# lbcb-sci/herro

Hardware: NVIDIA H100
Metric: corrected_bases_per_sec (higher is better)
Workload: dtype u8 pileup/consensus + f32 forward

## Files before the change

herro_b200/csrc/gemm_tc.cu:

```cuda
#include <cstdio>
#include <cuda.h>
#include <cuda_bf16.h>

#include "common.cuh"
#include "forward.h"

namespace hb {

namespace {

constexpr int BM = 128, BN = 128, BK = 64, STAGES = 3;
constexpr int STAGE_BYTES = (2 * BM + 2 * BN) * 128;
constexpr int C_THREADS = 256, G_THREADS = 288, G_PROD_WARP = 8;

__device__ __forceinline__ uint32_t smem_u32(const void* p) { return (uint32_t)__cvta_generic_to_shared(p); }

__device__ __forceinline__ void mbar_init(uint64_t* bar, uint32_t count) {
    asm volatile("mbarrier.init.shared::cta.b64 [%0], %1;" ::"r"(smem_u32(bar)), "r"(count));
}
__device__ __forceinline__ void mbar_arrive(uint64_t* bar) {
    asm volatile("{\n\t.reg .b64 st;\n\tmbarrier.arrive.shared::cta.b64 st, [%0];\n\t}" ::"r"(smem_u32(bar)) : "memory");
}
__device__ __forceinline__ void mbar_wait(uint64_t* bar, uint32_t parity) {
    asm volatile(
        "{\n\t"
        ".reg .pred p;\n\t"
        "WAIT_LOOP:\n\t"
        "mbarrier.try_wait.parity.shared::cta.b64 p, [%0], %1;\n\t"
        "@p bra WAIT_DONE;\n\t"
        "bra WAIT_LOOP;\n\t"
        "WAIT_DONE:\n\t"
        "}" ::"r"(smem_u32(bar)), "r"(parity)
        : "memory");
}
__device__ __forceinline__ void mbar_arrive_expect_tx(uint64_t* bar, uint32_t bytes) {
    asm volatile("mbarrier.arrive.expect_tx.shared::cta.b64 _, [%0], %1;" ::"r"(smem_u32(bar)), "r"(bytes) : "memory");
}
__device__ __forceinline__ void tma_load_2d(uint32_t dst, const CUtensorMap* tm, uint64_t* bar, int c_inner, int c_row) {
    asm volatile("cp.async.bulk.tensor.2d.shared::cluster.global.mbarrier::complete_tx::bytes [%0], [%1, {%3, %4}], [%2];" ::"r"(dst),
                 "l"((uint64_t)tm), "r"(smem_u32(bar)), "r"(c_inner), "r"(c_row)
                 : "memory");
}
__device__ __forceinline__ void bar_sync(int id, int n) { asm volatile("bar.sync %0, %1;" ::"r"(id), "r"(n) : "memory"); }
__device__ __forceinline__ void fence_async_smem() { asm volatile("fence.proxy.async.shared::cta;" ::: "memory"); }

__device__ __forceinline__ uint64_t make_desc(uint32_t saddr) {
    uint64_t d = 0;
    d |= (uint64_t)((saddr & 0x3ffffu) >> 4);
    d |= (uint64_t)1 << 16;
    d |= (uint64_t)(1024u >> 4) << 32;
    d |= (uint64_t)1 << 62;
    return d;
}

__device__ __forceinline__ void wg_fence() { asm volatile("wgmma.fence.sync.aligned;" ::: "memory"); }
__device__ __forceinline__ void wg_commit() { asm volatile("wgmma.commit_group.sync.aligned;" ::: "memory"); }
template <int N>
__device__ __forceinline__ void wg_wait() { asm volatile("wgmma.wait_group.sync.aligned %0;" ::"n"(N) : "memory"); }
template <int R>
__device__ __forceinline__ void acc_fence(float (&a)[R]) {
#pragma unroll
    for (int i = 0; i < R; i++) asm volatile("" : "+f"(a[i])::"memory");
}

__device__ __forceinline__ void wgmma_n128(float (&d)[64], uint64_t adesc, uint64_t bdesc, uint32_t accumulate) {
    asm volatile(
        "{\n\t.reg .pred p;\n\tsetp.ne.b32 p, %66, 0;\n\t"
        "wgmma.mma_async.sync.aligned.m64n128k16.f32.bf16.bf16 "
        "{%0, %1, %2, %3, %4, %5, %6, %7, %8, %9, %10, %11, %12, %13, %14, %15, %16, %17, %18, %19, %20, %21, %22, %23, %24, %25, %26, %27, %28, %29, %30, %31, %32, %33, %34, %35, %36, %37, %38, %39, %40, %41, %42, %43, %44, %45, %46, %47, %48, %49, %50, %51, %52, %53, %54, %55, %56, %57, %58, %59, %60, %61, %62, %63}, "
        "%64, %65, p, 1, 1, 0, 0;\n\t}"
        : "+f"(d[0]), "+f"(d[1]), "+f"(d[2]), "+f"(d[3]), "+f"(d[4]), "+f"(d[5]), "+f"(d[6]), "+f"(d[7]), "+f"(d[8]), "+f"(d[9]), "+f"(d[10]), "+f"(d[11]), "+f"(d[12]), "+f"(d[13]), "+f"(d[14]), "+f"(d[15]), "+f"(d[16]), "+f"(d[17]), "+f"(d[18]), "+f"(d[19]), "+f"(d[20]), "+f"(d[21]), "+f"(d[22]), "+f"(d[23]), "+f"(d[24]), "+f"(d[25]), "+f"(d[26]), "+f"(d[27]), "+f"(d[28]), "+f"(d[29]), "+f"(d[30]), "+f"(d[31]), "+f"(d[32]), "+f"(d[33]), "+f"(d[34]), "+f"(d[35]), "+f"(d[36]), "+f"(d[37]), "+f"(d[38]), "+f"(d[39]), "+f"(d[40]), "+f"(d[41]), "+f"(d[42]), "+f"(d[43]), "+f"(d[44]), "+f"(d[45]), "+f"(d[46]), "+f"(d[47]), "+f"(d[48]), "+f"(d[49]), "+f"(d[50]), "+f"(d[51]), "+f"(d[52]), "+f"(d[53]), "+f"(d[54]), "+f"(d[55]), "+f"(d[56]), "+f"(d[57]), "+f"(d[58]), "+f"(d[59]), "+f"(d[60]), "+f"(d[61]), "+f"(d[62]), "+f"(d[63])
        : "l"(adesc), "l"(bdesc), "r"(accumulate)
        : "memory");
}
__device__ __forceinline__ void wgmma_n96(float (&d)[48], uint64_t adesc, uint64_t bdesc, uint32_t accumulate) {
    asm volatile(
        "{\n\t.reg .pred p;\n\tsetp.ne.b32 p, %50, 0;\n\t"
        "wgmma.mma_async.sync.aligned.m64n96k16.f32.bf16.bf16 "
        "{%0, %1, %2, %3, %4, %5, %6, %7, %8, %9, %10, %11, %12, %13, %14, %15, %16, %17, %18, %19, %20, %21, %22, %23, %24, %25, %26, %27, %28, %29, %30, %31, %32, %33, %34, %35, %36, %37, %38, %39, %40, %41, %42, %43, %44, %45, %46, %47}, "
        "%48, %49, p, 1, 1, 0, 0;\n\t}"
        : "+f"(d[0]), "+f"(d[1]), "+f"(d[2]), "+f"(d[3]), "+f"(d[4]), "+f"(d[5]), "+f"(d[6]), "+f"(d[7]), "+f"(d[8]), "+f"(d[9]), "+f"(d[10]), "+f"(d[11]), "+f"(d[12]), "+f"(d[13]), "+f"(d[14]), "+f"(d[15]), "+f"(d[16]), "+f"(d[17]), "+f"(d[18]), "+f"(d[19]), "+f"(d[20]), "+f"(d[21]), "+f"(d[22]), "+f"(d[23]), "+f"(d[24]), "+f"(d[25]), "+f"(d[26]), "+f"(d[27]), "+f"(d[28]), "+f"(d[29]), "+f"(d[30]), "+f"(d[31]), "+f"(d[32]), "+f"(d[33]), "+f"(d[34]), "+f"(d[35]), "+f"(d[36]), "+f"(d[37]), "+f"(d[38]), "+f"(d[39]), "+f"(d[40]), "+f"(d[41]), "+f"(d[42]), "+f"(d[43]), "+f"(d[44]), "+f"(d[45]), "+f"(d[46]), "+f"(d[47])
        : "l"(adesc), "l"(bdesc), "r"(accumulate)
        : "memory");
}

__device__ __forceinline__ void mma_kblock(float (&acc)[64], uint32_t a_hi, uint32_t a_lo, uint32_t b_hi, uint32_t b_lo, bool zero) {
    const uint64_t dAh = make_desc(a_hi), dAl = make_desc(a_lo), dBh = make_desc(b_hi), dBl = make_desc(b_lo);
    wg_fence();
#pragma unroll
    for (int k = 0; k < BK / 16; k++) {
        const uint64_t adv = (uint64_t)(k * 2);
        wgmma_n128(acc, dAh + adv, dBh + adv, (zero && k == 0) ? 0u : 1u);
        wgmma_n128(acc, dAl + adv, dBh + adv, 1u);
        wgmma_n128(acc, dAh + adv, dBl + adv, 1u);
    }
    wg_commit();
}

__device__ __forceinline__ void split2(float a, float b, uint32_t& hi, uint32_t& lo) {
    const __nv_bfloat162 h = __floats2bfloat162_rn(a, b);
    hi = *reinterpret_cast<const uint32_t*>(&h);
    const float ah = __uint_as_float(hi << 16), bh = __uint_as_float(hi & 0xffff0000u);
    const __nv_bfloat162 l = __floats2bfloat162_rn(a - ah, b - bh);
    lo = *reinterpret_cast<const uint32_t*>(&l);
}

__device__ __forceinline__ void frag_ln_stats(const float (&a)[64], float& m0, float& r0, float& m1, float& r1) {
    float s0 = 0.f, s1 = 0.f;
#pragma unroll
    for (int j = 0; j < 16; j++) { s0 += a[4 * j] + a[4 * j + 1]; s1 += a[4 * j + 2] + a[4 * j + 3]; }
    s0 += __shfl_xor_sync(HB_FULL, s0, 1); s0 += __shfl_xor_sync(HB_FULL, s0, 2);
    s1 += __shfl_xor_sync(HB_FULL, s1, 1); s1 += __shfl_xor_sync(HB_FULL, s1, 2);
    m0 = s0 * (1.f / BN); m1 = s1 * (1.f / BN);
    float v0 = 0.f, v1 = 0.f;
#pragma unroll
    for (int j = 0; j < 16; j++) {
        float d = a[4 * j] - m0; v0 = fmaf(d, d, v0);
        d = a[4 * j + 1] - m0; v0 = fmaf(d, d, v0);
        d = a[4 * j + 2] - m1; v1 = fmaf(d, d, v1);
        d = a[4 * j + 3] - m1; v1 = fmaf(d, d, v1);
    }
    v0 += __shfl_xor_sync(HB_FULL, v0, 1); v0 += __shfl_xor_sync(HB_FULL, v0, 2);
    v1 += __shfl_xor_sync(HB_FULL, v1, 1); v1 += __shfl_xor_sync(HB_FULL, v1, 2);
    r0 = rsqrtf(v0 * (1.f / BN) + 1e-5f); r1 = rsqrtf(v1 * (1.f / BN) + 1e-5f);
}
__device__ __forceinline__ void frag_layernorm(float (&a)[64], const float* gam, const float* bet, int fc) {
    float m0, r0, m1, r1;
    frag_ln_stats(a, m0, r0, m1, r1);
#pragma unroll
    for (int j = 0; j < 16; j++) {
        const int c = 8 * j + fc;
        const float g0 = gam[c], g1 = gam[c + 1], b0 = bet[c], b1 = bet[c + 1];
        a[4 * j] = (a[4 * j] - m0) * r0 * g0 + b0;
        a[4 * j + 1] = (a[4 * j + 1] - m0) * r0 * g1 + b1;
        a[4 * j + 2] = (a[4 * j + 2] - m1) * r1 * g0 + b0;
        a[4 * j + 3] = (a[4 * j + 3] - m1) * r1 * g1 + b1;
    }
}
__device__ __forceinline__ void frag_store_f32(const float (&a)[64], float* base, size_t ld, size_t row0, int c0, int fc) {
#pragma unroll
    for (int j = 0; j < 16; j++) {
        *(float2*)(base + row0 * ld + c0 + 8 * j + fc) = make_float2(a[4 * j], a[4 * j + 1]);
        *(float2*)(base + (row0 + 8) * ld + c0 + 8 * j + fc) = make_float2(a[4 * j + 2], a[4 * j + 3]);
    }
}
__device__ __forceinline__ void frag_store_split(const float (&a)[64], __nv_bfloat16* hi, __nv_bfloat16* lo, size_t ld, size_t row0, int c0,
                                                 int fc) {
#pragma unroll
    for (int j = 0; j < 16; j++) {
        uint32_t h, l;
        const size_t o0 = row0 * ld + c0 + 8 * j + fc, o1 = (row0 + 8) * ld + c0 + 8 * j + fc;
        split2(a[4 * j], a[4 * j + 1], h, l);
        *(uint32_t*)(hi + o0) = h; *(uint32_t*)(lo + o0) = l;
        split2(a[4 * j + 2], a[4 * j + 3], h, l);
        *(uint32_t*)(hi + o1) = h; *(uint32_t*)(lo + o1) = l;
    }
}
__device__ __forceinline__ void frag_store_tile(const float (&a)[64], uint8_t* tile, int r, int fc, const float* gam = nullptr,
                                                const float* bet = nullptr, const float* ln = nullptr) {
#pragma unroll
    for (int j = 0; j < 16; j++)
#pragma unroll
        for (int hf = 0; hf < 2; hf++) {
            const int rr = r + 8 * hf, c = 8 * j + fc;
            float x = a[4 * j + 2 * hf], y = a[4 * j + 2 * hf + 1];
            if (gam) {
                x = (x - ln[2 * hf]) * ln[2 * hf + 1] * gam[c] + bet[c];
                y = (y - ln[2 * hf]) * ln[2 * hf + 1] * gam[c + 1] + bet[c + 1];
            }
            uint32_t h, l;
            split2(x, y, h, l);
            const uint32_t off = (uint32_t)(j >> 3) * (2 * BM * 128) + (uint32_t)rr * 128u + (uint32_t)((((j & 7) ^ (rr & 7)) << 4) + fc * 2);
            *(uint32_t*)(tile + off) = h;
            *(uint32_t*)(tile + off + BM * 128) = l;
        }
}

}

__global__ void __launch_bounds__(G_THREADS, 1) k_gemm_ws(GemmArgs g, const __grid_constant__ CUtensorMap tmAhi,
                                                         const __grid_constant__ CUtensorMap tmAlo, const __grid_constant__ CUtensorMap tmWhi,
                                                         const __grid_constant__ CUtensorMap tmWlo) {
    extern __shared__ uint8_t smem_dyn[];
    uint8_t* smem = smem_dyn + ((1024u - (smem_u32(smem_dyn) & 1023u)) & 1023u);
    __shared__ uint64_t full_bar[STAGES], empty_bar[STAGES];
    __shared__ __align__(16) float s_lng[BN], s_lnb[BN];

    const int tid = threadIdx.x, warp = tid >> 5, lane = tid & 31;
    if (tid == 0) {
        for (int s = 0; s < STAGES; s++) { mbar_init(&full_bar[s], 1); mbar_init(&empty_bar[s], C_THREADS); }
        asm volatile("fence.mbarrier_init.release.cluster;" ::: "memory");
    }
    if (g.mode == GEMM_OUT_F32_RES_LN && tid < BN) { s_lng[tid] = g.ln_g[tid]; s_lnb[tid] = g.ln_b[tid]; }
    __syncthreads();

    const uint32_t n_items = g.m_tiles * g.n_chunks;
    const uint32_t kbs = g.k_blocks;

    if (warp == G_PROD_WARP) {
        if (lane == 0) {
            uint32_t it_stage = 0;
            for (uint32_t item = blockIdx.x; item < n_items; item += gridDim.x) {
                const int m0 = (int)((item / g.n_chunks) * BM), n0 = (int)((item % g.n_chunks) * BN);
                for (uint32_t kb = 0; kb < kbs; kb++, it_stage++) {
                    const uint32_t s = it_stage % STAGES, ph = (it_stage / STAGES) & 1;
                    mbar_wait(&empty_bar[s], ph ^ 1);
                    const uint32_t sb = smem_u32(smem + (size_t)s * STAGE_BYTES);
                    const int k0 = (int)(kb * BK);
                    mbar_arrive_expect_tx(&full_bar[s], STAGE_BYTES);
                    tma_load_2d(sb, &tmAhi, &full_bar[s], k0, m0);
                    tma_load_2d(sb + BM * 128, &tmAlo, &full_bar[s], k0, m0);
                    tma_load_2d(sb + 2 * BM * 128, &tmWhi, &full_bar[s], k0, n0);
                    tma_load_2d(sb + 2 * BM * 128 + BN * 128, &tmWlo, &full_bar[s], k0, n0);
                }
            }
        }
        return;
    }
    const int wg = warp >> 2;
    const int fr = wg * 64 + (warp & 3) * 16 + (lane >> 2), fc = (lane & 3) * 2;
    uint32_t it_stage = 0;
    float acc[64];
    for (uint32_t item = blockIdx.x; item < n_items; item += gridDim.x) {
        const uint32_t m0 = (item / g.n_chunks) * BM, n0 = (item % g.n_chunks) * BN;
        uint32_t prev = 0;
        for (uint32_t kb = 0; kb < kbs; kb++, it_stage++) {
            const uint32_t s = it_stage % STAGES, ph = (it_stage / STAGES) & 1;
            mbar_wait(&full_bar[s], ph);
            const uint32_t sb = smem_u32(smem + (size_t)s * STAGE_BYTES);
            mma_kblock(acc, sb + wg * 64 * 128, sb + BM * 128 + wg * 64 * 128, sb + 2 * BM * 128, sb + 2 * BM * 128 + BN * 128, kb == 0);
            if (kb > 0) {
                wg_wait<1>();
                mbar_arrive(&empty_bar[prev]);
            }
            prev = s;
        }
        wg_wait<0>();
        acc_fence(acc);
        mbar_arrive(&empty_bar[prev]);
        const size_t row0 = (size_t)m0 + fr;
        if (g.mode == GEMM_OUT_F32_RES_LN) {
#pragma unroll
            for (int j = 0; j < 16; j++) {
                const int c = 8 * j + fc;
                const float2 bv = *(const float2*)(g.bias + c);
                const float2 x0 = *(const float2*)(g.res + row0 * g.ldc + c), x1 = *(const float2*)(g.res + (row0 + 8) * g.ldc + c);
                acc[4 * j] = acc[4 * j] + bv.x + x0.x; acc[4 * j + 1] = acc[4 * j + 1] + bv.y + x0.y;
                acc[4 * j + 2] = acc[4 * j + 2] + bv.x + x1.x; acc[4 * j + 3] = acc[4 * j + 3] + bv.y + x1.y;
            }
            frag_store_f32(acc, g.out, g.ldc, row0, 0, fc);
            frag_layernorm(acc, s_lng, s_lnb, fc);
            frag_store_split(acc, g.out_hi, g.out_lo, g.ldo, row0, 0, fc);
            continue;
        }
#pragma unroll
        for (int j = 0; j < 16; j++) {
            const int c = (int)n0 + 8 * j + fc;
            const float2 bv = *(const float2*)(g.bias + c);
            acc[4 * j] += bv.x; acc[4 * j + 1] += bv.y; acc[4 * j + 2] += bv.x; acc[4 * j + 3] += bv.y;
            if (g.mode == GEMM_OUT_F32_RES) {
                const float2 x0 = *(const float2*)(g.res + row0 * g.ldc + c), x1 = *(const float2*)(g.res + (row0 + 8) * g.ldc + c);
                acc[4 * j] += x0.x; acc[4 * j + 1] += x0.y; acc[4 * j + 2] += x1.x; acc[4 * j + 3] += x1.y;
            } else if (g.mode == GEMM_OUT_F32_RELU || g.mode == GEMM_OUT_SPLIT_RELU) {
#pragma unroll
                for (int e = 0; e < 4; e++) acc[4 * j + e] = fmaxf(acc[4 * j + e], 0.f);
            }
        }
        if (g.mode == GEMM_OUT_SPLIT_RELU) frag_store_split(acc, g.out_hi, g.out_lo, g.ldo, row0, (int)n0, fc);
        else frag_store_f32(acc, g.out, g.ldc, row0, (int)n0, fc);
    }
}

constexpr int FFN_RING_BYTES = 2 * BN * 128;
constexpr int FFN_A_BYTES = 2 * 2 * BM * 128;
constexpr int FFN_STAGES = 2;

template <bool FUSE_O>
__global__ void __launch_bounds__(G_THREADS, 1) k_ffn_ws(FfnArgs g, const __grid_constant__ CUtensorMap tmHhi,
                                                        const __grid_constant__ CUtensorMap tmHlo, const __grid_constant__ CUtensorMap tmW1hi,
                                                        const __grid_constant__ CUtensorMap tmW1lo, const __grid_constant__ CUtensorMap tmW2hi,
                                                        const __grid_constant__ CUtensorMap tmW2lo, const __grid_constant__ CUtensorMap tmWohi,
                                                        const __grid_constant__ CUtensorMap tmWolo) {
    extern __shared__ uint8_t smem_dyn[];
    uint8_t* smem = smem_dyn + ((1024u - (smem_u32(smem_dyn) & 1023u)) & 1023u);
    uint8_t* sA1 = smem;
    uint8_t* sA2 = sA1 + FFN_A_BYTES;
    uint8_t* ring = sA2 + FFN_A_BYTES;
    __shared__ uint64_t full_bar[FFN_STAGES], empty_bar[FFN_STAGES], a1_full, a1_empty;
    __shared__ __align__(16) float s_b1[512], s_b2[BN], s_lng[BN], s_lnb[BN], s_bo[BN], s_ln2g[BN], s_ln2b[BN];

    const int tid = threadIdx.x, warp = tid >> 5, lane = tid & 31;
    if (tid == 0) {
        for (int s = 0; s < FFN_STAGES; s++) { mbar_init(&full_bar[s], 1); mbar_init(&empty_bar[s], C_THREADS); }
        mbar_init(&a1_full, 1); mbar_init(&a1_empty, C_THREADS);
        asm volatile("fence.mbarrier_init.release.cluster;" ::: "memory");
    }
    for (int i = tid; i < 512; i += G_THREADS) s_b1[i] = g.b1[i];
    if (tid < BN) { s_b2[tid] = g.b2[tid]; s_lng[tid] = g.ln_g[tid]; s_lnb[tid] = g.ln_b[tid]; }
    if (FUSE_O && tid < BN) { s_bo[tid] = g.bo[tid]; s_ln2g[tid] = g.ln2_g[tid]; s_ln2b[tid] = g.ln2_b[tid]; }
    __syncthreads();

    if (warp == G_PROD_WARP) {
        if (lane == 0) {
            uint32_t it_stage = 0, n_done = 0;
            auto load_w = [&](const CUtensorMap* hi, const CUtensorMap* lo, int col, int row) {
                const uint32_t s = it_stage % FFN_STAGES, ph = (it_stage / FFN_STAGES) & 1;
                mbar_wait(&empty_bar[s], ph ^ 1);
                const uint32_t sb = smem_u32(ring + (size_t)s * FFN_RING_BYTES);
                mbar_arrive_expect_tx(&full_bar[s], FFN_RING_BYTES);
                tma_load_2d(sb, hi, &full_bar[s], col, row);
                tma_load_2d(sb + BN * 128, lo, &full_bar[s], col, row);
                it_stage++;
            };
            for (uint32_t tile = blockIdx.x; tile < g.m_tiles; tile += gridDim.x, n_done++) {
                mbar_wait(&a1_empty, (n_done & 1) ^ 1);
                mbar_arrive_expect_tx(&a1_full, FFN_A_BYTES);
                for (int kb = 0; kb < 2; kb++) {
                    tma_load_2d(smem_u32(sA1) + kb * (2 * BM * 128), &tmHhi, &a1_full, kb * BK, (int)(tile * BM));
                    tma_load_2d(smem_u32(sA1) + kb * (2 * BM * 128) + BM * 128, &tmHlo, &a1_full, kb * BK, (int)(tile * BM));
                }
                if (FUSE_O)
                    for (int kb = 0; kb < 2; kb++) load_w(&tmWohi, &tmWolo, kb * BK, 0);
                for (int c = 0; c < 4; c++) {
                    for (int kb = 0; kb < 2; kb++) load_w(&tmW1hi, &tmW1lo, kb * BK, c * 128);
                    for (int kb = 0; kb < 2; kb++) load_w(&tmW2hi, &tmW2lo, c * 128 + kb * BK, 0);
                }
            }
        }
        return;
    }
    const int wg = warp >> 2;
    const int fr = wg * 64 + (warp & 3) * 16 + (lane >> 2), fc = (lane & 3) * 2;
    const uint32_t a1b = smem_u32(sA1) + wg * 64 * 128, a2b = smem_u32(sA2) + wg * 64 * 128;
    uint32_t it_stage = 0, n_done = 0;
    float accO[64], accF[64];
    auto contract = [&](float (&acc)[64], uint32_t abase, bool zero) {
        for (int kb = 0; kb < 2; kb++, it_stage++) {
            const uint32_t s = it_stage % FFN_STAGES, ph = (it_stage / FFN_STAGES) & 1;
            mbar_wait(&full_bar[s], ph);
            const uint32_t sb = smem_u32(ring + (size_t)s * FFN_RING_BYTES);
            const uint32_t a = abase + kb * (2 * BM * 128);
            mma_kblock(acc, a, a + BM * 128, sb, sb + BN * 128, zero && kb == 0);
        }
        wg_wait<0>();
        acc_fence(acc);
        mbar_arrive(&empty_bar[(it_stage - 2) % FFN_STAGES]);
        mbar_arrive(&empty_bar[(it_stage - 1) % FFN_STAGES]);
    };
    for (uint32_t tile = blockIdx.x; tile < g.m_tiles; tile += gridDim.x, n_done++) {
        const size_t row0 = (size_t)tile * BM + fr;
        if (!FUSE_O) {
#pragma unroll
            for (int j = 0; j < 16; j++) {
                const int c = 8 * j + fc;
                const float2 x0 = *(const float2*)(g.X + row0 * BN + c), x1 = *(const float2*)(g.X + (row0 + 8) * BN + c);
                accO[4 * j] = x0.x + s_b2[c]; accO[4 * j + 1] = x0.y + s_b2[c + 1];
                accO[4 * j + 2] = x1.x + s_b2[c]; accO[4 * j + 3] = x1.y + s_b2[c + 1];
            }
        }
        mbar_wait(&a1_full, n_done & 1);
        if (FUSE_O) {
            contract(accO, a1b, true);
#pragma unroll
            for (int j = 0; j < 16; j++) {
                const int c = 8 * j + fc;
                const float2 x0 = *(const float2*)(g.X + row0 * BN + c), x1 = *(const float2*)(g.X + (row0 + 8) * BN + c);
                accO[4 * j] = accO[4 * j] + s_bo[c] + x0.x; accO[4 * j + 1] = accO[4 * j + 1] + s_bo[c + 1] + x0.y;
                accO[4 * j + 2] = accO[4 * j + 2] + s_bo[c] + x1.x; accO[4 * j + 3] = accO[4 * j + 3] + s_bo[c + 1] + x1.y;
            }
            float ln[4];
            frag_ln_stats(accO, ln[0], ln[1], ln[2], ln[3]);
            bar_sync(1 + wg, 128);
            frag_store_tile(accO, sA1, fr, fc, s_ln2g, s_ln2b, ln);
#pragma unroll
            for (int j = 0; j < 16; j++) {
                const int c = 8 * j + fc;
                accO[4 * j] += s_b2[c]; accO[4 * j + 1] += s_b2[c + 1]; accO[4 * j + 2] += s_b2[c]; accO[4 * j + 3] += s_b2[c + 1];
            }
            fence_async_smem();
            bar_sync(1 + wg, 128);
        }
        for (int c = 0; c < 4; c++) {
            contract(accF, a1b, true);
            if (c == 3) mbar_arrive(&a1_empty);
#pragma unroll
            for (int j = 0; j < 16; j++) {
                const float b0 = s_b1[c * 128 + 8 * j + fc], b1 = s_b1[c * 128 + 8 * j + fc + 1];
                accF[4 * j] = fmaxf(accF[4 * j] + b0, 0.f); accF[4 * j + 1] = fmaxf(accF[4 * j + 1] + b1, 0.f);
                accF[4 * j + 2] = fmaxf(accF[4 * j + 2] + b0, 0.f); accF[4 * j + 3] = fmaxf(accF[4 * j + 3] + b1, 0.f);
            }
            frag_store_tile(accF, sA2, fr, fc);
            fence_async_smem();
            bar_sync(1 + wg, 128);
            contract(accO, a2b, false);
            bar_sync(1 + wg, 128);
        }
        if (g.store_x) frag_store_f32(accO, g.X, BN, row0, 0, fc);
        frag_layernorm(accO, s_lng, s_lnb, fc);
        frag_store_split(accO, g.out_hi, g.out_lo, BN, row0, 0, fc);
    }
}

constexpr int QA_HROWS = 96;
constexpr int QA_RING_BYTES = 2 * QA_HROWS * 128;
constexpr int QA_STAGES = 3;
constexpr int QA_POS_BYTES = 6 * 2048;

__device__ __forceinline__ void ldsm_x4(uint32_t addr, uint32_t (&r)[4]) {
    asm volatile("ldmatrix.sync.aligned.m8n8.x4.shared.b16 {%0, %1, %2, %3}, [%4];" : "=r"(r[0]), "=r"(r[1]), "=r"(r[2]), "=r"(r[3]) : "r"(addr));
}
__device__ __forceinline__ void ldsm_x4_trans(uint32_t addr, uint32_t (&r)[4]) {
    asm volatile("ldmatrix.sync.aligned.m8n8.x4.trans.shared.b16 {%0, %1, %2, %3}, [%4];" : "=r"(r[0]), "=r"(r[1]), "=r"(r[2]), "=r"(r[3]) : "r"(addr));
}
__device__ __forceinline__ void mma16816(float (&c)[4], const uint32_t (&a)[4], uint32_t b0, uint32_t b1) {
    asm volatile("mma.sync.aligned.m16n8k16.row.col.f32.bf16.bf16.f32 {%0, %1, %2, %3}, {%4, %5, %6, %7}, {%8, %9}, {%0, %1, %2, %3};"
                 : "+f"(c[0]), "+f"(c[1]), "+f"(c[2]), "+f"(c[3])
                 : "r"(a[0]), "r"(a[1]), "r"(a[2]), "r"(a[3]), "r"(b0), "r"(b1));
}
__device__ __forceinline__ uint32_t qa_off(int row, int chunk) { return (uint32_t)(row * 64 + ((chunk ^ ((row >> 1) & 3)) << 4)); }

__global__ void __launch_bounds__(G_THREADS, 1) k_qkv_attn_ws(QkvAttnArgs g, const __grid_constant__ CUtensorMap tmHhi,
                                                             const __grid_constant__ CUtensorMap tmHlo, const __grid_constant__ CUtensorMap tmWhi,
                                                             const __grid_constant__ CUtensorMap tmWlo) {
    extern __shared__ uint8_t smem_dyn[];
    uint8_t* smem = smem_dyn + ((1024u - (smem_u32(smem_dyn) & 1023u)) & 1023u);
    uint8_t* sA = smem;
    uint8_t* ring = sA + FFN_A_BYTES;
    uint8_t* sP = ring + QA_STAGES * QA_RING_BYTES;
    __shared__ uint64_t full_bar[QA_STAGES], empty_bar[QA_STAGES], a_full, a_empty;
    __shared__ __align__(16) float s_bias[4 * QA_HROWS];

    const int tid = threadIdx.x, warp = tid >> 5, lane = tid & 31;
    if (tid == 0) {
        for (int s = 0; s < QA_STAGES; s++) { mbar_init(&full_bar[s], 1); mbar_init(&empty_bar[s], C_THREADS); }
        mbar_init(&a_full, 1); mbar_init(&a_empty, C_THREADS);
        asm volatile("fence.mbarrier_init.release.cluster;" ::: "memory");
    }
    for (int i = tid; i < 4 * QA_HROWS; i += G_THREADS) s_bias[i] = g.bias[i];
    __syncthreads();

    if (warp == G_PROD_WARP) {
        if (lane == 0) {
            uint32_t it_stage = 0, n_done = 0;
            for (uint32_t tile = blockIdx.x; tile < g.m_tiles; tile += gridDim.x, n_done++) {
                const int m0 = (int)(tile * BM);
                mbar_wait(&a_empty, (n_done & 1) ^ 1);
                mbar_arrive_expect_tx(&a_full, FFN_A_BYTES);
                for (int kb = 0; kb < 2; kb++) {
                    tma_load_2d(smem_u32(sA) + kb * (2 * BM * 128), &tmHhi, &a_full, kb * BK, m0);
                    tma_load_2d(smem_u32(sA) + kb * (2 * BM * 128) + BM * 128, &tmHlo, &a_full, kb * BK, m0);
                }
                for (int h = 0; h < 4; h++)
                    for (int kb = 0; kb < 2; kb++, it_stage++) {
                        const uint32_t s = it_stage % QA_STAGES, ph = (it_stage / QA_STAGES) & 1;
                        mbar_wait(&empty_bar[s], ph ^ 1);
                        const uint32_t sb = smem_u32(ring + (size_t)s * QA_RING_BYTES);
                        mbar_arrive_expect_tx(&full_bar[s], QA_RING_BYTES);
                        tma_load_2d(sb, &tmWhi, &full_bar[s], kb * BK, h * QA_HROWS);
                        tma_load_2d(sb + QA_HROWS * 128, &tmWlo, &full_bar[s], kb * BK, h * QA_HROWS);
                    }
            }
        }
        return;
    }
    const int wg = warp >> 2;
    const int pos = wg * 2 + ((warp & 3) >> 1);
    const int mt = warp & 1;
    const int gq = lane >> 2, tq = lane & 3;
    uint8_t* pb = sP + (size_t)pos * QA_POS_BYTES;
    uint8_t *aQh = pb, *aQl = pb + 2048, *aKh = pb + 4096, *aKl = pb + 6144, *aVh = pb + 8192, *aVl = pb + 10240;
    const uint32_t uQh = smem_u32(aQh), uQl = smem_u32(aQl), uKh = smem_u32(aKh), uKl = smem_u32(aKl), uVh = smem_u32(aVh),
                   uVl = smem_u32(aVl);
    const float scale_l2 = rsqrtf(32.f) * 1.4426950408889634f;
    const uint32_t ab = smem_u32(sA) + wg * 64 * 128;
    uint32_t it_stage = 0, n_done = 0;
    for (uint32_t tile = blockIdx.x; tile < g.m_tiles; tile += gridDim.x, n_done++) {
        mbar_wait(&a_full, n_done & 1);
        for (int h = 0; h < 4; h++) {
            float acc[48];
            for (int kb = 0; kb < 2; kb++, it_stage++) {
                const uint32_t s = it_stage % QA_STAGES, ph = (it_stage / QA_STAGES) & 1;
                mbar_wait(&full_bar[s], ph);
                const uint32_t sb = smem_u32(ring + (size_t)s * QA_RING_BYTES);
                const uint32_t a = ab + kb * (2 * BM * 128);
                const uint64_t dAh = make_desc(a), dAl = make_desc(a + BM * 128), dBh = make_desc(sb), dBl = make_desc(sb + QA_HROWS * 128);
                wg_fence();
#pragma unroll
                for (int k = 0; k < BK / 16; k++) {
                    const uint64_t adv = (uint64_t)(k * 2);
                    wgmma_n96(acc, dAh + adv, dBh + adv, (kb | k) ? 1u : 0u);
                    wgmma_n96(acc, dAl + adv, dBh + adv, 1u);
                    wgmma_n96(acc, dAh + adv, dBl + adv, 1u);
                }
                wg_commit();
            }
            wg_wait<0>();
            acc_fence(acc);
            mbar_arrive(&empty_bar[(it_stage - 2) % QA_STAGES]);
            mbar_arrive(&empty_bar[(it_stage - 1) % QA_STAGES]);
            if (h == 3) mbar_arrive(&a_empty);
            bar_sync(3 + pos, 64);
            const float* bb = s_bias + h * QA_HROWS;
#pragma unroll
            for (int j = 0; j < 12; j++) {
                const int c = 8 * j + 2 * tq;
                const float sc = j < 4 ? scale_l2 : 1.f;
                uint8_t* hi_arr = j < 4 ? aQh : (j < 8 ? aKh : aVh);
                const int cc = c & 31;
#pragma unroll
                for (int hf = 0; hf < 2; hf++) {
                    const int row = mt * 16 + hf * 8 + gq;
                    uint32_t hw, lw;
                    split2((acc[4 * j + 2 * hf] + bb[c]) * sc, (acc[4 * j + 2 * hf + 1] + bb[c + 1]) * sc, hw, lw);
                    const uint32_t off = qa_off(row, cc >> 3) + (cc & 7) * 2;
                    *(uint32_t*)(hi_arr + off) = hw;
                    *(uint32_t*)(hi_arr + 2048 + off) = lw;
                }
            }
            bar_sync(3 + pos, 64);
            float sacc[4][4];
#pragma unroll
            for (int nt = 0; nt < 4; nt++)
#pragma unroll
                for (int e = 0; e < 4; e++) sacc[nt][e] = 0.f;
            {
                uint32_t qh[2][4], ql[2][4];
#pragma unroll
                for (int ks = 0; ks < 2; ks++) {
                    const uint32_t off = qa_off(mt * 16 + (lane & 7) + ((lane >> 3) & 1) * 8, ks * 2 + (lane >> 4));
                    ldsm_x4(uQh + off, qh[ks]);
                    ldsm_x4(uQl + off, ql[ks]);
                }
#pragma unroll
                for (int ntp = 0; ntp < 2; ntp++)
#pragma unroll
                    for (int ks = 0; ks < 2; ks++) {
                        uint32_t kh[4], kl[4];
                        const uint32_t off = qa_off(ntp * 16 + (lane & 7) + (lane >> 4) * 8, ks * 2 + ((lane >> 3) & 1));
                        ldsm_x4(uKh + off, kh);
                        ldsm_x4(uKl + off, kl);
#pragma unroll
                        for (int j = 0; j < 2; j++) {
                            mma16816(sacc[ntp * 2 + j], qh[ks], kh[2 * j], kh[2 * j + 1]);
                            mma16816(sacc[ntp * 2 + j], ql[ks], kh[2 * j], kh[2 * j + 1]);
                            mma16816(sacc[ntp * 2 + j], qh[ks], kl[2 * j], kl[2 * j + 1]);
                        }
                    }
            }
            float inv[2];
// ... 164 lines not shown
    if (warp >= S_GATHER_WARP) {
        const int gt = tid - S_GATHER_WARP * 32;
        uint32_t n_done = 0;
        for (uint32_t item = blockIdx.x; item < n_items; item += gridDim.x, n_done++) {
            uint8_t* tb = tokbuf + (n_done & 1) * 4 * STEM_MAXK * 32;
            uint8_t* qb = qbuf + (n_done & 1) * 4 * STEM_MAXK * 32;
            uint32_t m_row = 0, m_L = 0, m_Lref = 0;
            uint64_t m_base = 0;
            if (lane < 4 && item * 4 + lane < g.npos) {
                const uint32_t w = b.fwd_win[g.n0 + item * 4 + lane];
                m_row = b.fwd_row[g.n0 + item * 4 + lane];
                m_L = b.w_L[w]; m_Lref = b.w_reflmax[w]; m_base = b.w_rowbase[w];
            }
            mbar_wait(&buf_empty[n_done & 1], ((n_done >> 1) & 1) ^ 1);
            for (int i0 = 0; i0 < 4 * K * 2; i0 += S_GATHER) {
                const int i = i0 + gt;
                const int ps = min(i / (K * 2), 3), rem = i % (K * 2), j = rem >> 1, half = rem & 1;
                const uint32_t r = __shfl_sync(HB_FULL, m_row, ps), L = __shfl_sync(HB_FULL, m_L, ps), Lref = __shfl_sync(HB_FULL, m_Lref, ps);
                const uint64_t rbase = __shfl_sync(HB_FULL, m_base, ps);
                uint4 tv = make_uint4(0xffffffffu, 0xffffffffu, 0xffffffffu, 0xffffffffu), qv = make_uint4(0, 0, 0, 0);
                const int64_t row = (int64_t)r + j - K / 2;
                if (row >= 0 && row < (int64_t)Lref) {
                    if (row < (int64_t)L) {
                        const uint64_t off = (rbase + row) * ROW_BYTES + half * 16;
                        tv = *(const uint4*)(b.mat_bases + off);
                        qv = *(const uint4*)(b.mat_quals + off);
                    } else {
                        tv = make_uint4(0x0b0b0b0bu, 0x0b0b0b0bu, 0x0b0b0b0bu, 0x0b0b0b0bu);
                        qv = make_uint4(0x7e7e7e7eu, 0x7e7e7e7eu, 0x7e7e7e7eu, 0x7e7e7e7eu);
                    }
                }
                if (i < 4 * K * 2) {
                    *(uint4*)(tb + (ps * STEM_MAXK + j) * 32 + half * 16) = tv;
                    *(uint4*)(qb + (ps * STEM_MAXK + j) * 32 + half * 16) = qv;
                }
            }
            mbar_arrive(&buf_full[n_done & 1]);
        }
        return;
    }
    const int wg = warp >> 2;
    const int fr = wg * 64 + (warp & 3) * 16 + (lane >> 2), fc = (lane & 3) * 2;
    const int rd0 = fr & 31, rd1 = (fr + 8) & 31;
    uint32_t it_stage = 0;
    float acc[64];
    for (uint32_t item = blockIdx.x; item < n_items; item += gridDim.x) {
        uint32_t prev = 0;
        for (uint32_t kb = 0; kb < kbs; kb++, it_stage++) {
            const uint32_t s = it_stage % STAGES, ph = (it_stage / STAGES) & 1;
            mbar_wait(&full_bar[s], ph);
            const uint32_t sb = smem_u32(smem + (size_t)s * STEM_STAGE_BYTES);
            const uint64_t dA = make_desc(sb + wg * 64 * 128), dBh = make_desc(sb + BM * 128), dBl = make_desc(sb + BM * 128 + BN * 128);
            wg_fence();
#pragma unroll
            for (int k = 0; k < BK / 16; k++) {
                const uint64_t adv = (uint64_t)(k * 2);
                wgmma_n128(acc, dA + adv, dBh + adv, (kb | (uint32_t)k) ? 1u : 0u);
                wgmma_n128(acc, dA + adv, dBl + adv, 1u);
            }
            wg_commit();
            if (kb > 0) {
                wg_wait<1>();
                mbar_arrive(&empty_bar[prev]);
            }
            prev = s;
        }
        wg_wait<0>();
        acc_fence(acc);
        mbar_arrive(&empty_bar[prev]);
        const size_t row0 = (size_t)item * BM + fr;
#pragma unroll
        for (int j = 0; j < 16; j++) {
            const int c = 8 * j + fc;
            const float* rp0 = s_rp + rd0 * STEM_RP_LD + c;
            const float* rp1 = s_rp + rd1 * STEM_RP_LD + c;
            acc[4 * j] = fmaxf(acc[4 * j] + s_bias[c], 0.f) + rp0[0];
            acc[4 * j + 1] = fmaxf(acc[4 * j + 1] + s_bias[c + 1], 0.f) + rp0[1];
            acc[4 * j + 2] = fmaxf(acc[4 * j + 2] + s_bias[c], 0.f) + rp1[0];
            acc[4 * j + 3] = fmaxf(acc[4 * j + 3] + s_bias[c + 1], 0.f) + rp1[1];
            if (rd0 >= R_COLS) { acc[4 * j] = 0.f; acc[4 * j + 1] = 0.f; }
            if (rd1 >= R_COLS) { acc[4 * j + 2] = 0.f; acc[4 * j + 3] = 0.f; }
        }
        frag_store_f32(acc, g.X, BN, row0, 0, fc);
        if (g.out_hi) {
            frag_layernorm(acc, s_lng, s_lnb, fc);
            frag_store_split(acc, g.out_hi, g.out_lo, BN, row0, 0, fc);
        }
    }
}

__global__ void k_split_bf16(const float* __restrict__ w, __nv_bfloat16* __restrict__ hi, __nv_bfloat16* __restrict__ lo, size_t n) {
    const size_t i = (size_t)blockIdx.x * blockDim.x + threadIdx.x;
    if (i < n) {
        const __nv_bfloat16 h = __float2bfloat16_rn(w[i]);
        hi[i] = h;
        lo[i] = __float2bfloat16_rn(w[i] - __bfloat162float(h));
    }
}

cudaError_t split_weights(const float* w, size_t n, void** hi, void** lo) {
    cudaError_t e = cudaMalloc(hi, n * 2);
    if (e != cudaSuccess) return e;
    e = cudaMalloc(lo, n * 2);
    if (e != cudaSuccess) return e;
    k_split_bf16<<<(unsigned)((n + 255) / 256), 256>>>(w, (__nv_bfloat16*)*hi, (__nv_bfloat16*)*lo, n);
    return cudaGetLastError();
}

typedef CUresult (*EncodeTiledFn)(CUtensorMap*, CUtensorMapDataType, cuuint32_t, void*, const cuuint64_t*, const cuuint64_t*,
                                  const cuuint32_t*, const cuuint32_t*, CUtensorMapInterleave, CUtensorMapSwizzle,
                                  CUtensorMapL2promotion, CUtensorMapFloatOOBfill);
static EncodeTiledFn encode_fn() {
    static EncodeTiledFn fn = nullptr;
    if (!fn) {
        void* p = nullptr;
        cudaDriverEntryPointQueryResult q;
        if (cudaGetDriverEntryPoint("cuTensorMapEncodeTiled", &p, cudaEnableDefault, &q) == cudaSuccess) fn = (EncodeTiledFn)p;
    }
    return fn;
}
static bool make_tmap(CUtensorMap* tm, const void* base, uint64_t rows, uint64_t cols, uint64_t ld, uint32_t box_rows = BM) {
    EncodeTiledFn fn = encode_fn();
    if (!fn) return false;
    const cuuint64_t gdim[2] = {cols, rows};
    const cuuint64_t gstr[1] = {ld * 2};
    const cuuint32_t box[2] = {BK, box_rows};
    const cuuint32_t estr[2] = {1, 1};
    return fn(tm, CU_TENSOR_MAP_DATA_TYPE_BFLOAT16, 2, const_cast<void*>(base), gdim, gstr, box, estr, CU_TENSOR_MAP_INTERLEAVE_NONE,
              CU_TENSOR_MAP_SWIZZLE_128B, CU_TENSOR_MAP_L2_PROMOTION_L2_128B, CU_TENSOR_MAP_FLOAT_OOB_FILL_NONE) == CUDA_SUCCESS;
}

cudaError_t gemm_tc(const GemmArgs& a, int num_sms, cudaStream_t st) {
    static bool configured = false;
    const size_t smem = (size_t)STAGES * STAGE_BYTES + 1024;
    if (!configured) {
        cudaError_t e = cudaFuncSetAttribute(k_gemm_ws, cudaFuncAttributeMaxDynamicSharedMemorySize, (int)smem);
        if (e != cudaSuccess) return e;
        configured = true;
    }
    const uint32_t items = a.m_tiles * a.n_chunks;
    if (items == 0) return cudaSuccess;
    CUtensorMap tAh, tAl, tWh, tWl;
    const uint64_t M = (uint64_t)a.m_tiles * BM, N = (uint64_t)a.n_chunks * BN;
    if (!make_tmap(&tAh, a.Ahi, M, a.K, a.lda) || !make_tmap(&tAl, a.Alo, M, a.K, a.lda) || !make_tmap(&tWh, a.Whi, N, a.K, a.K) ||
        !make_tmap(&tWl, a.Wlo, N, a.K, a.K))
        return cudaErrorInvalidValue;
    const unsigned grid = (unsigned)std::min<uint32_t>(items, (uint32_t)num_sms);
    k_gemm_ws<<<grid, G_THREADS, smem, st>>>(a, tAh, tAl, tWh, tWl);
    return cudaGetLastError();
}

cudaError_t ffn_tc(const FfnArgs& a, int num_sms, cudaStream_t st) {
    static bool configured = false;
    const size_t smem = (size_t)2 * FFN_A_BYTES + (size_t)FFN_STAGES * FFN_RING_BYTES + 1024;
    if (!configured) {
        cudaError_t e = cudaFuncSetAttribute(k_ffn_ws<false>, cudaFuncAttributeMaxDynamicSharedMemorySize, (int)smem);
        if (e != cudaSuccess) return e;
        e = cudaFuncSetAttribute(k_ffn_ws<true>, cudaFuncAttributeMaxDynamicSharedMemorySize, (int)smem);
        if (e != cudaSuccess) return e;
        configured = true;
    }
    if (a.m_tiles == 0) return cudaSuccess;
    CUtensorMap tHh, tHl, t1h, t1l, t2h, t2l, toh, tol;
    const uint64_t T = (uint64_t)a.m_tiles * BM;
    if (!make_tmap(&tHh, a.Hhi, T, BN, BN) || !make_tmap(&tHl, a.Hlo, T, BN, BN) || !make_tmap(&t1h, a.W1hi, a.F, BN, BN) ||
        !make_tmap(&t1l, a.W1lo, a.F, BN, BN) || !make_tmap(&t2h, a.W2hi, BN, a.F, a.F) || !make_tmap(&t2l, a.W2lo, BN, a.F, a.F))
        return cudaErrorInvalidValue;
    const unsigned grid = (unsigned)std::min<uint32_t>(a.m_tiles, (uint32_t)num_sms);
    if (a.Wohi) {
        if (!make_tmap(&toh, a.Wohi, BN, BN, BN) || !make_tmap(&tol, a.Wolo, BN, BN, BN)) return cudaErrorInvalidValue;
        k_ffn_ws<true><<<grid, G_THREADS, smem, st>>>(a, tHh, tHl, t1h, t1l, t2h, t2l, toh, tol);
    } else {
        k_ffn_ws<false><<<grid, G_THREADS, smem, st>>>(a, tHh, tHl, t1h, t1l, t2h, t2l, t1h, t1l);
    }
    return cudaGetLastError();
}

cudaError_t stem_tc(const BatchView& b, const StemArgs& a, int num_sms, cudaStream_t st) {
    static bool configured = false;
    const size_t smem = (size_t)STAGES * STEM_STAGE_BYTES + 2 * 2 * 4 * STEM_MAXK * 32 + (size_t)32 * STEM_RP_LD * 4 + 1024;
    if (!configured) {
        cudaError_t e = cudaFuncSetAttribute(k_stem_tc, cudaFuncAttributeMaxDynamicSharedMemorySize, (int)smem);
        if (e != cudaSuccess) return e;
        configured = true;
    }
    const uint32_t items = (a.npos + 3) / 4;
    if (items == 0) return cudaSuccess;
    CUtensorMap tWh, tWl;
    if (!make_tmap(&tWh, a.Whi, BN, a.Kp, a.Kp) || !make_tmap(&tWl, a.Wlo, BN, a.Kp, a.Kp)) return cudaErrorInvalidValue;
    k_stem_tc<<<(unsigned)std::min<uint32_t>(items, (uint32_t)num_sms), S_THREADS, smem, st>>>(b, a, tWh, tWl);
    return cudaGetLastError();
}

cudaError_t qkv_attn_tc(const QkvAttnArgs& a, int num_sms, cudaStream_t st) {
    static bool configured = false;
    const size_t smem = (size_t)FFN_A_BYTES + (size_t)QA_STAGES * QA_RING_BYTES + (size_t)4 * QA_POS_BYTES + 1024;
    if (!configured) {
        cudaError_t e = cudaFuncSetAttribute(k_qkv_attn_ws, cudaFuncAttributeMaxDynamicSharedMemorySize, (int)smem);
        if (e != cudaSuccess) return e;
        configured = true;
    }
    if (a.m_tiles == 0) return cudaSuccess;
    CUtensorMap tHh, tHl, tWh, tWl;
    const uint64_t T = (uint64_t)a.m_tiles * BM;
    if (!make_tmap(&tHh, a.Hhi, T, BN, BN) || !make_tmap(&tHl, a.Hlo, T, BN, BN) || !make_tmap(&tWh, a.Whi, 4 * QA_HROWS, BN, BN, QA_HROWS) ||
        !make_tmap(&tWl, a.Wlo, 4 * QA_HROWS, BN, BN, QA_HROWS))
        return cudaErrorInvalidValue;
    k_qkv_attn_ws<<<(unsigned)std::min<uint32_t>(a.m_tiles, (uint32_t)num_sms), G_THREADS, smem, st>>>(a, tHh, tHl, tWh, tWl);
    return cudaGetLastError();
}

}
```

Before: 488.5 million.

## Keep FFN hidden activations in registers and overlap wgmma chunks in fused FFN

The fused FFN kernel now holds the ReLU'd hidden chunk as bf16 hi/lo register fragments and feeds them to register-A wgmma, instead of staging it through a second shared-memory tile with barriers. The next W1 chunk's wgmma is issued while the W2 contraction is in flight, and ring slots are retired incrementally. The weight ring grows to four stages, a producer warpgroup with setmaxnreg register rebalancing is added, and residual X is loaded once per tile. This removes smem round-trips and serialization, but adds register pressure (240 regs per consumer) and more complex async ordering.

```diff
diff --git a/herro_b200/csrc/gemm_tc.cu b/herro_b200/csrc/gemm_tc.cu
--- a/herro_b200/csrc/gemm_tc.cu
+++ b/herro_b200/csrc/gemm_tc.cu
@@ -73,6 +73,15 @@
         : "l"(adesc), "l"(bdesc), "r"(accumulate)
         : "memory");
 }
+__device__ __forceinline__ void wgmma_n128_ra(float (&d)[64], uint32_t a0, uint32_t a1, uint32_t a2, uint32_t a3, uint64_t bdesc) {
+    asm volatile(
+        "wgmma.mma_async.sync.aligned.m64n128k16.f32.bf16.bf16 "
+        "{%0, %1, %2, %3, %4, %5, %6, %7, %8, %9, %10, %11, %12, %13, %14, %15, %16, %17, %18, %19, %20, %21, %22, %23, %24, %25, %26, %27, %28, %29, %30, %31, %32, %33, %34, %35, %36, %37, %38, %39, %40, %41, %42, %43, %44, %45, %46, %47, %48, %49, %50, %51, %52, %53, %54, %55, %56, %57, %58, %59, %60, %61, %62, %63}, "
+        "{%64, %65, %66, %67}, %68, 1, 1, 1, 0;"
+        : "+f"(d[0]), "+f"(d[1]), "+f"(d[2]), "+f"(d[3]), "+f"(d[4]), "+f"(d[5]), "+f"(d[6]), "+f"(d[7]), "+f"(d[8]), "+f"(d[9]), "+f"(d[10]), "+f"(d[11]), "+f"(d[12]), "+f"(d[13]), "+f"(d[14]), "+f"(d[15]), "+f"(d[16]), "+f"(d[17]), "+f"(d[18]), "+f"(d[19]), "+f"(d[20]), "+f"(d[21]), "+f"(d[22]), "+f"(d[23]), "+f"(d[24]), "+f"(d[25]), "+f"(d[26]), "+f"(d[27]), "+f"(d[28]), "+f"(d[29]), "+f"(d[30]), "+f"(d[31]), "+f"(d[32]), "+f"(d[33]), "+f"(d[34]), "+f"(d[35]), "+f"(d[36]), "+f"(d[37]), "+f"(d[38]), "+f"(d[39]), "+f"(d[40]), "+f"(d[41]), "+f"(d[42]), "+f"(d[43]), "+f"(d[44]), "+f"(d[45]), "+f"(d[46]), "+f"(d[47]), "+f"(d[48]), "+f"(d[49]), "+f"(d[50]), "+f"(d[51]), "+f"(d[52]), "+f"(d[53]), "+f"(d[54]), "+f"(d[55]), "+f"(d[56]), "+f"(d[57]), "+f"(d[58]), "+f"(d[59]), "+f"(d[60]), "+f"(d[61]), "+f"(d[62]), "+f"(d[63])
+        : "r"(a0), "r"(a1), "r"(a2), "r"(a3), "l"(bdesc)
+        : "memory");
+}
 __device__ __forceinline__ void wgmma_n96(float (&d)[48], uint64_t adesc, uint64_t bdesc, uint32_t accumulate) {
     asm volatile(
         "{\n\t.reg .pred p;\n\tsetp.ne.b32 p, %50, 0;\n\t"
@@ -95,6 +104,25 @@
         wgmma_n128(acc, dAh + adv, dBl + adv, 1u);
     }
     wg_commit();
+}
+__device__ __forceinline__ void mma_kblock_ra(float (&acc)[64], const uint32_t (&ah)[32], const uint32_t (&al)[32], int kb, uint32_t b_hi,
+                                              uint32_t b_lo) {
+    const uint64_t dBh = make_desc(b_hi), dBl = make_desc(b_lo);
+    wg_fence();
+#pragma unroll
+    for (int k = 0; k < BK / 16; k++) {
+        const uint64_t adv = (uint64_t)(k * 2);
+        const int s = 4 * (4 * kb + k);
+        wgmma_n128_ra(acc, ah[s], ah[s + 1], ah[s + 2], ah[s + 3], dBh + adv);
+        wgmma_n128_ra(acc, al[s], al[s + 1], al[s + 2], al[s + 3], dBh + adv);
+        wgmma_n128_ra(acc, ah[s], ah[s + 1], ah[s + 2], ah[s + 3], dBl + adv);
+    }
+    wg_commit();
+}
+template <int R>
+__device__ __forceinline__ void reg_fence(uint32_t (&a)[R]) {
+#pragma unroll
+    for (int i = 0; i < R; i++) asm volatile("" : "+r"(a[i])::"memory");
 }
 
 __device__ __forceinline__ void split2(float a, float b, uint32_t& hi, uint32_t& lo) {
@@ -273,10 +301,18 @@
 
 constexpr int FFN_RING_BYTES = 2 * BN * 128;
 constexpr int FFN_A_BYTES = 2 * 2 * BM * 128;
-constexpr int FFN_STAGES = 2;
+constexpr int FFN_STAGES = 4;
+constexpr int FFN_THREADS = 384, FFN_PROD_WARP = 8, FFN_PROD_REGS = 24, FFN_CONS_REGS = 240;
+
+template <int N>
+__device__ __forceinline__ void ffn_retire(uint64_t* empty_bar, uint32_t it_stage) {
+    wg_wait<N>();
+    mbar_arrive(&empty_bar[(it_stage - 1 - N) % FFN_STAGES]);
+    if constexpr (N > 0) ffn_retire<N - 1>(empty_bar, it_stage);
+}
 
 template <bool FUSE_O>
-__global__ void __launch_bounds__(G_THREADS, 1) k_ffn_ws(FfnArgs g, const __grid_constant__ CUtensorMap tmHhi,
+__global__ void __launch_bounds__(FFN_THREADS, 1) k_ffn_ws(FfnArgs g, const __grid_constant__ CUtensorMap tmHhi,
                                                         const __grid_constant__ CUtensorMap tmHlo, const __grid_constant__ CUtensorMap tmW1hi,
                                                         const __grid_constant__ CUtensorMap tmW1lo, const __grid_constant__ CUtensorMap tmW2hi,
                                                         const __grid_constant__ CUtensorMap tmW2lo, const __grid_constant__ CUtensorMap tmWohi,
@@ -284,8 +320,7 @@
     extern __shared__ uint8_t smem_dyn[];
     uint8_t* smem = smem_dyn + ((1024u - (smem_u32(smem_dyn) & 1023u)) & 1023u);
     uint8_t* sA1 = smem;
-    uint8_t* sA2 = sA1 + FFN_A_BYTES;
-    uint8_t* ring = sA2 + FFN_A_BYTES;
+    uint8_t* ring = sA1 + FFN_A_BYTES;
     __shared__ uint64_t full_bar[FFN_STAGES], empty_bar[FFN_STAGES], a1_full, a1_empty;
     __shared__ __align__(16) float s_b1[512], s_b2[BN], s_lng[BN], s_lnb[BN], s_bo[BN], s_ln2g[BN], s_ln2b[BN];
 
@@ -295,13 +330,14 @@
         mbar_init(&a1_full, 1); mbar_init(&a1_empty, C_THREADS);
         asm volatile("fence.mbarrier_init.release.cluster;" ::: "memory");
     }
-    for (int i = tid; i < 512; i += G_THREADS) s_b1[i] = g.b1[i];
+    for (int i = tid; i < 512; i += FFN_THREADS) s_b1[i] = g.b1[i];
     if (tid < BN) { s_b2[tid] = g.b2[tid]; s_lng[tid] = g.ln_g[tid]; s_lnb[tid] = g.ln_b[tid]; }
     if (FUSE_O && tid < BN) { s_bo[tid] = g.bo[tid]; s_ln2g[tid] = g.ln2_g[tid]; s_ln2b[tid] = g.ln2_b[tid]; }
     __syncthreads();
 
-    if (warp == G_PROD_WARP) {
-        if (lane == 0) {
+    if (warp >= FFN_PROD_WARP) {
+        asm volatile("setmaxnreg.dec.sync.aligned.u32 %0;" ::"n"(FFN_PROD_REGS));
+        if (warp == FFN_PROD_WARP && lane == 0) {
             uint32_t it_stage = 0, n_done = 0;
             auto load_w = [&](const CUtensorMap* hi, const CUtensorMap* lo, int col, int row) {
                 const uint32_t s = it_stage % FFN_STAGES, ph = (it_stage / FFN_STAGES) & 1;
@@ -329,42 +365,64 @@
         }
         return;
     }
+    asm volatile("setmaxnreg.inc.sync.aligned.u32 %0;" ::"n"(FFN_CONS_REGS));
     const int wg = warp >> 2;
     const int fr = wg * 64 + (warp & 3) * 16 + (lane >> 2), fc = (lane & 3) * 2;
-    const uint32_t a1b = smem_u32(sA1) + wg * 64 * 128, a2b = smem_u32(sA2) + wg * 64 * 128;
+    const uint32_t a1b = smem_u32(sA1) + wg * 64 * 128;
     uint32_t it_stage = 0, n_done = 0;
     float accO[64], accF[64];
-    auto contract = [&](float (&acc)[64], uint32_t abase, bool zero) {
+    uint32_t ahi[32], alo[32];
+    auto issue = [&](float (&acc)[64], int kb, bool zero) {
+        const uint32_t s = it_stage % FFN_STAGES, ph = (it_stage / FFN_STAGES) & 1;
+        mbar_wait(&full_bar[s], ph);
+        const uint32_t sb = smem_u32(ring + (size_t)s * FFN_RING_BYTES), a = a1b + kb * (2 * BM * 128);
+        mma_kblock(acc, a, a + BM * 128, sb, sb + BN * 128, zero && kb == 0);
+        it_stage++;
+    };
+    auto issue_f2 = [&]() {
+#pragma unroll
         for (int kb = 0; kb < 2; kb++, it_stage++) {
             const uint32_t s = it_stage % FFN_STAGES, ph = (it_stage / FFN_STAGES) & 1;
             mbar_wait(&full_bar[s], ph);
             const uint32_t sb = smem_u32(ring + (size_t)s * FFN_RING_BYTES);
-            const uint32_t a = abase + kb * (2 * BM * 128);
-            mma_kblock(acc, a, a + BM * 128, sb, sb + BN * 128, zero && kb == 0);
-        }
-        wg_wait<0>();
-        acc_fence(acc);
-        mbar_arrive(&empty_bar[(it_stage - 2) % FFN_STAGES]);
-        mbar_arrive(&empty_bar[(it_stage - 1) % FFN_STAGES]);
+            mma_kblock_ra(accO, ahi, alo, kb, sb, sb + BN * 128);
+        }
+    };
+    auto e1 = [&](int c) {
+#pragma unroll
+        for (int j = 0; j < 16; j++) {
+            const float b0 = s_b1[c * 128 + 8 * j + fc], b1 = s_b1[c * 128 + 8 * j + fc + 1];
+            split2(fmaxf(accF[4 * j] + b0, 0.f), fmaxf(accF[4 * j + 1] + b1, 0.f), ahi[2 * j], alo[2 * j]);
+            split2(fmaxf(accF[4 * j + 2] + b0, 0.f), fmaxf(accF[4 * j + 3] + b1, 0.f), ahi[2 * j + 1], alo[2 * j + 1]);
+        }
     };
     for (uint32_t tile = blockIdx.x; tile < g.m_tiles; tile += gridDim.x, n_done++) {
         const size_t row0 = (size_t)tile * BM + fr;
+        float2 xr[32];
+#pragma unroll
+        for (int j = 0; j < 16; j++) {
+            xr[2 * j] = *(const float2*)(g.X + row0 * BN + 8 * j + fc);
+            xr[2 * j + 1] = *(const float2*)(g.X + (row0 + 8) * BN + 8 * j + fc);
+        }
         if (!FUSE_O) {
 #pragma unroll
             for (int j = 0; j < 16; j++) {
                 const int c = 8 * j + fc;
-                const float2 x0 = *(const float2*)(g.X + row0 * BN + c), x1 = *(const float2*)(g.X + (row0 + 8) * BN + c);
+                const float2 x0 = xr[2 * j], x1 = xr[2 * j + 1];
                 accO[4 * j] = x0.x + s_b2[c]; accO[4 * j + 1] = x0.y + s_b2[c + 1];
                 accO[4 * j + 2] = x1.x + s_b2[c]; accO[4 * j + 3] = x1.y + s_b2[c + 1];
             }
         }
         mbar_wait(&a1_full, n_done & 1);
         if (FUSE_O) {
-            contract(accO, a1b, true);
+            issue(accO, 0, true);
+            issue(accO, 1, true);
+            ffn_retire<1>(empty_bar, it_stage);
+            acc_fence(accO);
 #pragma unroll
             for (int j = 0; j < 16; j++) {
                 const int c = 8 * j + fc;
-                const float2 x0 = *(const float2*)(g.X + row0 * BN + c), x1 = *(const float2*)(g.X + (row0 + 8) * BN + c);
+                const float2 x0 = xr[2 * j], x1 = xr[2 * j + 1];
                 accO[4 * j] = accO[4 * j] + s_bo[c] + x0.x; accO[4 * j + 1] = accO[4 * j + 1] + s_bo[c + 1] + x0.y;
                 accO[4 * j + 2] = accO[4 * j + 2] + s_bo[c] + x1.x; accO[4 * j + 3] = accO[4 * j + 3] + s_bo[c + 1] + x1.y;
             }
@@ -380,21 +438,27 @@
             fence_async_smem();
             bar_sync(1 + wg, 128);
         }
-        for (int c = 0; c < 4; c++) {
-            contract(accF, a1b, true);
-            if (c == 3) mbar_arrive(&a1_empty);
-#pragma unroll
-            for (int j = 0; j < 16; j++) {
-                const float b0 = s_b1[c * 128 + 8 * j + fc], b1 = s_b1[c * 128 + 8 * j + fc + 1];
-                accF[4 * j] = fmaxf(accF[4 * j] + b0, 0.f); accF[4 * j + 1] = fmaxf(accF[4 * j + 1] + b1, 0.f);
-                accF[4 * j + 2] = fmaxf(accF[4 * j + 2] + b0, 0.f); accF[4 * j + 3] = fmaxf(accF[4 * j + 3] + b1, 0.f);
-            }
-            frag_store_tile(accF, sA2, fr, fc);
-            fence_async_smem();
-            bar_sync(1 + wg, 128);
-            contract(accO, a2b, false);
-            bar_sync(1 + wg, 128);
-        }
+        issue(accF, 0, true);
+        issue(accF, 1, true);
+        ffn_retire<1>(empty_bar, it_stage);
+        acc_fence(accF);
+        e1(0);
+        for (int c = 0; c < 3; c++) {
+            issue_f2();
+            issue(accF, 0, true);
+            issue(accF, 1, true);
+            ffn_retire<3>(empty_bar, it_stage);
+            acc_fence(accF);
+            reg_fence(ahi);
+            reg_fence(alo);
+            if (c == 2) mbar_arrive(&a1_empty);
+            e1(c + 1);
+        }
+        issue_f2();
+        ffn_retire<1>(empty_bar, it_stage);
+        acc_fence(accO);
+        reg_fence(ahi);
+        reg_fence(alo);
         if (g.store_x) frag_store_f32(accO, g.X, BN, row0, 0, fc);
         frag_layernorm(accO, s_lng, s_lnb, fc);
         frag_store_split(accO, g.out_hi, g.out_lo, BN, row0, 0, fc);
@@ -865,7 +929,7 @@
 
 cudaError_t ffn_tc(const FfnArgs& a, int num_sms, cudaStream_t st) {
     static bool configured = false;
-    const size_t smem = (size_t)2 * FFN_A_BYTES + (size_t)FFN_STAGES * FFN_RING_BYTES + 1024;
+    const size_t smem = (size_t)FFN_A_BYTES + (size_t)FFN_STAGES * FFN_RING_BYTES + 1024;
     if (!configured) {
         cudaError_t e = cudaFuncSetAttribute(k_ffn_ws<false>, cudaFuncAttributeMaxDynamicSharedMemorySize, (int)smem);
         if (e != cudaSuccess) return e;
@@ -882,9 +946,9 @@
     const unsigned grid = (unsigned)std::min<uint32_t>(a.m_tiles, (uint32_t)num_sms);
     if (a.Wohi) {
         if (!make_tmap(&toh, a.Wohi, BN, BN, BN) || !make_tmap(&tol, a.Wolo, BN, BN, BN)) return cudaErrorInvalidValue;
-        k_ffn_ws<true><<<grid, G_THREADS, smem, st>>>(a, tHh, tHl, t1h, t1l, t2h, t2l, toh, tol);
+        k_ffn_ws<true><<<grid, FFN_THREADS, smem, st>>>(a, tHh, tHl, t1h, t1l, t2h, t2l, toh, tol);
     } else {
-        k_ffn_ws<false><<<grid, G_THREADS, smem, st>>>(a, tHh, tHl, t1h, t1l, t2h, t2l, t1h, t1l);
+        k_ffn_ws<false><<<grid, FFN_THREADS, smem, st>>>(a, tHh, tHl, t1h, t1l, t2h, t2l, t1h, t1l);
     }
     return cudaGetLastError();
 }
```

Measured after the change: 539.7 million (median of 6 runs). 10.5% higher.
